# jianzhangcs/DAGL

Hardware: AMD Instinct MI355X
Metric: graph-attn fwd query-patches/s @256x256x64 k=8 (higher is better)
Workload: dtype f32

## Files before the change

### dagl_amd/csrc/aggregate.hip

```cpp
#include "dagl_common.h"
#include "aggregate_direct.h"
#include "topk_merge.h"

namespace dagl {


__global__ __launch_bounds__(256) void edge_softmax_fast_kernel(EdgeArgs a) {
    const int lane = threadIdx.x & 63;
    const size_t ql = (size_t)blockIdx.x * 4 + (threadIdx.x >> 6);
    if (ql >= (size_t)a.B * a.L) return;
    int n = a.cnt[ql];
    if (n > DAGL_FAST_CAP) n = DAGL_FAST_CAP;
    int key = 0x7fffffff; float s = 0.f;
    if (lane < n) { key = a.list_idx[ql * DAGL_FAST_CAP + lane]; s = a.list_val[ql * DAGL_FAST_CAP + lane]; }
#pragma unroll
    for (int k2 = 2; k2 <= 64; k2 <<= 1) {
#pragma unroll
        for (int j = k2 >> 1; j > 0; j >>= 1) {
            const int okey = __shfl_xor(key, j);
            const float os = __shfl_xor(s, j);
            const bool up = ((lane & k2) == 0);
            const bool lower = ((lane & j) == 0);
            const bool take = (lower == up) ? (okey < key) : (okey > key);
            if (take) { key = okey; s = os; }
// ... 52 lines not shown
__global__ void row_stats_kernel(size_t n_rows, const float* __restrict__ nb_wgt, const int32_t* __restrict__ nb_cnt,
                                 const int64_t* __restrict__ row_off, int width, int32_t* __restrict__ deg,
                                 float* __restrict__ rowsum) {
    const size_t r = (size_t)blockIdx.x * blockDim.x + threadIdx.x;
    if (r >= n_rows) return;
    const int n = nb_cnt[r];
    if (n < 0) return;
    const float* w = nb_wgt + (row_off ? (size_t)row_off[r] : r * width);
    double s = 0.0;
    for (int j = 0; j < n; ++j) s += (double)w[j];
    if (deg) deg[r] = n;
    if (rowsum) rowsum[r] = (float)s;
}

int launch_row_stats(hipStream_t s, size_t n_rows, const float* nb_wgt, const int32_t* nb_cnt, const int64_t* row_off,
                     int width, int32_t* deg, float* rowsum) {
    hipLaunchKernelGGL(row_stats_kernel, dim3((unsigned)((n_rows + 255) / 256)), dim3(256), 0, s, n_rows, nb_wgt,
                       nb_cnt, row_off, width, deg, rowsum);
    DAGL_LAUNCH_CHECK("row_stats_kernel");
    return DAGL_OK;
}

int launch_edge_softmax(hipStream_t s, const EdgeArgs& a) {
    const size_t nq = (size_t)a.B * a.L;
    dim3 grid((unsigned)((nq + 3) / 4)), block(256);
    if (a.mode == DAGL_MODE_ADAPTIVE) {
        if (a.row_off == nullptr) hipLaunchKernelGGL(edge_softmax_fast_kernel, grid, block, 0, s, a);
        else hipLaunchKernelGGL(edge_softmax_csr_kernel, grid, block, 0, s, a);
    } else {
        const int ks = topk_slots(a.k);
        if (a.splits * 2 * ks > TOPK_MAX_CAND) {
            set_error("edge softmax: %d candidates per query exceed %d", a.splits * 2 * ks, TOPK_MAX_CAND);
            return DAGL_ERR_INVALID;
        }
        dim3 g2 = grid;
        if (a.run_flags != nullptr && g2.x > 128) g2.x = 128;
        hipLaunchKernelGGL(edge_softmax_topk_kernel, g2, block, 0, s, a, ks, grid.x);
    }
    DAGL_LAUNCH_CHECK("edge_softmax_kernel");
    return DAGL_OK;
}

__global__ __launch_bounds__(256) void aggregate_direct_kernel(AggArgs a) {
    __shared__ int sh_of[AGG_STAGE];
    __shared__ float sh_w[AGG_STAGE];
    aggregate_direct_block(a, blockIdx.y, blockIdx.x, sh_of, sh_w);
}

int launch_aggregate_direct(hipStream_t s, const AggArgs& a) {
    dim3 grid((unsigned)a.g.L, a.B), block(256);
    hipLaunchKernelGGL(aggregate_direct_kernel, grid, block, 0, s, a);
    DAGL_LAUNCH_CHECK("aggregate_direct_kernel");
    return DAGL_OK;
}

template <int KU>
__global__ __launch_bounds__(256) void gather_rows_kernel(int L, int k, int P4, const int32_t* __restrict__ idx,
                                                          const float* __restrict__ wgt,
                                                          const float4* __restrict__ values,
                                                          float4* __restrict__ out) {
    const size_t t = (size_t)blockIdx.x * blockDim.x + threadIdx.x;
    if (t >= (size_t)L * P4) return;
    const int q = (int)(t / P4), r = (int)(t % P4);
    const int32_t* ip = idx + (size_t)q * k;
    const float* wp = wgt + (size_t)q * k;
    float4 acc = make_float4(0.f, 0.f, 0.f, 0.f);
    int j = 0;
    for (; j + KU <= k; j += KU) {
        int id[KU]; float w[KU]; float4 v[KU];
#pragma unroll
        for (int u = 0; u < KU; ++u) { id[u] = ip[j + u]; w[u] = wp[j + u]; }
#pragma unroll
        for (int u = 0; u < KU; ++u) {
            const bool ok = id[u] >= 0;
            v[u] = values[(size_t)(ok ? id[u] : 0) * P4 + r];
            if (!ok) w[u] = 0.f;
        }
#pragma unroll
        for (int u = 0; u < KU; ++u) {
            acc.x = fmaf(w[u], v[u].x, acc.x); acc.y = fmaf(w[u], v[u].y, acc.y);
            acc.z = fmaf(w[u], v[u].z, acc.z); acc.w = fmaf(w[u], v[u].w, acc.w);
        }
    }
    for (; j < k; ++j) {
        const int id = ip[j];
        if (id < 0) continue;
        const float w = wp[j];
        const float4 v = values[(size_t)id * P4 + r];
        acc.x = fmaf(w, v.x, acc.x); acc.y = fmaf(w, v.y, acc.y);
        acc.z = fmaf(w, v.z, acc.z); acc.w = fmaf(w, v.w, acc.w);
    }
    out[t] = acc;
}

int launch_gather_fixed(hipStream_t s, int L, int k, int P_, const int32_t* idx, const float* wgt,
                        const float* values, float* out) {
    const int P4 = P_ / 4;
    const size_t items = (size_t)L * P4;
    dim3 grid((unsigned)((items + 255) / 256)), block(256);
    if (k % 8 == 0)
        hipLaunchKernelGGL(gather_rows_kernel<8>, grid, block, 0, s, L, k, P4, idx, wgt,
                           reinterpret_cast<const float4*>(values), reinterpret_cast<float4*>(out));
    else
        hipLaunchKernelGGL(gather_rows_kernel<4>, grid, block, 0, s, L, k, P4, idx, wgt,
                           reinterpret_cast<const float4*>(values), reinterpret_cast<float4*>(out));
    DAGL_LAUNCH_CHECK("gather_rows_kernel");
    return DAGL_OK;
}

__global__ __launch_bounds__(256) void fold_kernel(Grid g, const float* __restrict__ agg, float* __restrict__ out,
                                                   int imgs, int heads, RangeTag range) {
    const int b = blockIdx.z;
    const int y = blockIdx.y;
    const int x = blockIdx.x * blockDim.x + threadIdx.x;
    const bool poisoned = (range.word != nullptr && *range.word == range.tag) || (range.veto != nullptr && *range.veto == range.tag);
    if (range.done != nullptr && b == 0 && y == 0 && blockIdx.x == 0 && threadIdx.x == 0) *range.done = range.tag;
    if (x >= g.W) return;
    int r0 = (y - 3 + QS - 1) / QS; if (y - 3 < 0) r0 = 0;
    int r1 = (y + 3) / QS; if (r1 > g.Lh - 1) r1 = g.Lh - 1;
    int c0 = (x - 3 + QS - 1) / QS; if (x - 3 < 0) c0 = 0;
    int c1 = (x + 3) / QS; if (c1 > g.Lw - 1) c1 = g.Lw - 1;
    float4 acc[CH / 4];
#pragma unroll
    for (int u = 0; u < CH / 4; ++u) acc[u] = make_float4(0.f, 0.f, 0.f, 0.f);
    for (int r = r0; r <= r1; ++r) {
        const int kh = y - (QS * r - 3);
        for (int c = c0; c <= c1; ++c) {
            const int kw = x - (QS * c - 3);
            const float4* p = reinterpret_cast<const float4*>(
                agg + ((size_t)b * g.L + (size_t)r * g.Lw + c) * P + (kh * KS + kw) * CH);
#pragma unroll
            for (int u = 0; u < CH / 4; ++u) {
                const float4 v = p[u];
                acc[u].x += v.x; acc[u].y += v.y; acc[u].z += v.z; acc[u].w += v.w;
            }
        }
    }
    float cnt = (float)((r1 - r0 + 1) * (c1 - c0 + 1));
    if (poisoned) cnt = __builtin_nanf("");
    const int head = b / imgs, img = b - head * imgs;
    float* o = out + ((size_t)img * heads + head) * CH * g.N + (size_t)y * g.W + x;
#pragma unroll
    for (int u = 0; u < CH / 4; ++u) {
        o[(size_t)(4 * u + 0) * g.N] = acc[u].x / cnt;
        o[(size_t)(4 * u + 1) * g.N] = acc[u].y / cnt;
        o[(size_t)(4 * u + 2) * g.N] = acc[u].z / cnt;
        o[(size_t)(4 * u + 3) * g.N] = acc[u].w / cnt;
    }
}

__device__ __forceinline__ void key_row_col(int id, int W, float inv_w, int& jy, int& jx) {
    jy = (int)((float)id * inv_w);
    jx = id - jy * W;
    if (jx < 0) { --jy; jx += W; } else if (jx >= W) { ++jy; jx -= W; }
}

__global__ __launch_bounds__(256) void aggregate_fold_kernel(AggArgs a, float* __restrict__ out, int imgs, int heads,
                                                             RangeTag range) {
    const Grid& g = a.g;
    const int b = blockIdx.z;
    const int t = blockIdx.x * blockDim.x + threadIdx.x;
    const int pix = t >> 2, u = t & 3;
    bool poisoned = range.word != nullptr && *range.word == range.tag;
    if (range.done != nullptr && b == 0 && blockIdx.x == 0 && threadIdx.x == 0) *range.done = range.tag;
    if (a.unserved != nullptr && *a.unserved != 0) {
        poisoned = true;
        if (b == 0 && blockIdx.x == 0 && threadIdx.x == 0) *a.unserved_sticky = 1;
    }
    if (pix >= g.N) return;
    const int y = pix / g.W, x = pix - y * g.W;
    int r0 = (y - 3 + QS - 1) / QS; if (y - 3 < 0) r0 = 0;
    int r1 = (y + 3) / QS; if (r1 > g.Lh - 1) r1 = g.Lh - 1;
    int c0 = (x - 3 + QS - 1) / QS; if (x - 3 < 0) c0 = 0;
    int c1 = (x + 3) / QS; if (c1 > g.Lw - 1) c1 = g.Lw - 1;
    const float4* vm = reinterpret_cast<const float4*>(a.b2p + (size_t)b * g.Hp * g.Wp * CH) + u;
    const int W = g.W, Wp = g.Wp;
    const float inv_w = 1.0f / (float)W;
    float4 acc = make_float4(0.f, 0.f, 0.f, 0.f);
    for (int r = r0; r <= r1; ++r) {
        const int kh = y - (QS * r - 3);
        for (int c = c0; c <= c1; ++c) {
            const int kw = x - (QS * c - 3);
            const size_t ql = (size_t)b * g.L + (size_t)r * g.Lw + c;
            const int n = a.nb_cnt[ql];
            const int32_t* ip = a.nb_idx + ql * a.width;
            const float* wp = a.nb_wgt + ql * a.width;
            float4 q = make_float4(0.f, 0.f, 0.f, 0.f);
            int j = 0;
            for (; j + 4 <= n; j += 4) {
                int id[4]; float w[4]; float4 v[4];
#pragma unroll
                for (int e = 0; e < 4; ++e) { id[e] = ip[j + e]; w[e] = wp[j + e]; }
#pragma unroll
                for (int e = 0; e < 4; ++e) {
                    int jy, jx; key_row_col(id[e], W, inv_w, jy, jx);
                    v[e] = vm[((jy + kh) * Wp + jx + kw) * (CH / 4)];
                }
#pragma unroll
                for (int e = 0; e < 4; ++e) {
                    q.x = fmaf(w[e], v[e].x, q.x); q.y = fmaf(w[e], v[e].y, q.y);
                    q.z = fmaf(w[e], v[e].z, q.z); q.w = fmaf(w[e], v[e].w, q.w);
                }
            }
            for (; j < n; ++j) {
                const int id = ip[j]; const float w = wp[j];
                int jy, jx; key_row_col(id, W, inv_w, jy, jx);
                const float4 v = vm[((jy + kh) * Wp + jx + kw) * (CH / 4)];
                q.x = fmaf(w, v.x, q.x); q.y = fmaf(w, v.y, q.y);
                q.z = fmaf(w, v.z, q.z); q.w = fmaf(w, v.w, q.w);
            }
            acc.x += q.x; acc.y += q.y; acc.z += q.z; acc.w += q.w;
        }
    }
    float cnt = (float)((r1 - r0 + 1) * (c1 - c0 + 1));
    if (poisoned) cnt = __builtin_nanf("");
    const int head = b / imgs, img = b - head * imgs;
    float* o = out + ((size_t)img * heads + head) * CH * g.N + (size_t)y * g.W + x;
    o[(size_t)(4 * u + 0) * g.N] = acc.x / cnt;
    o[(size_t)(4 * u + 1) * g.N] = acc.y / cnt;
    o[(size_t)(4 * u + 2) * g.N] = acc.z / cnt;
    o[(size_t)(4 * u + 3) * g.N] = acc.w / cnt;
}

int launch_aggregate_fold(hipStream_t s, const AggArgs& a, float* out, int heads, RangeTag range) {
    dim3 grid((unsigned)(((size_t)a.g.N * 4 + 255) / 256), 1, a.B), block(256);
    hipLaunchKernelGGL(aggregate_fold_kernel, grid, block, 0, s, a, out, a.B / heads, heads, range);
    DAGL_LAUNCH_CHECK("aggregate_fold_kernel");
    return DAGL_OK;
}

int launch_fold(hipStream_t s, int B, const Grid& g, const float* agg, float* out, int heads, RangeTag range) {
    dim3 grid((g.W + 63) / 64, g.H, B), block(64);
    hipLaunchKernelGGL(fold_kernel, grid, block, 0, s, g, agg, out, B / heads, heads, range);
    DAGL_LAUNCH_CHECK("fold_kernel");
    return DAGL_OK;
}

constexpr int MIX_TILES = 4;
__global__ __launch_bounds__(256) void stage_mix_kernel(int HW, const float* __restrict__ cat, const float* __restrict__ x,
                                                        const float* __restrict__ mix_w, const float* __restrict__ mix_b,
                                                        float* __restrict__ out) {
    const int lane = threadIdx.x & 63, wave = threadIdx.x >> 6;
    const int i = lane & 15, g = lane >> 4;
    const int b = blockIdx.y;
    const int pw = (blockIdx.x * 4 + wave) * (16 * MIX_TILES);
    if (pw >= HW) return;
    float w[4][16];
#pragma unroll
    for (int n = 0; n < 4; ++n)
#pragma unroll
        for (int T = 0; T < 16; ++T) w[n][T] = mix_w[(n * 16 + i) * 64 + 4 * T + g];
    float bo[4][4];
#pragma unroll
    for (int n = 0; n < 4; ++n)
#pragma unroll
        for (int r = 0; r < 4; ++r) bo[n][r] = mix_b[n * 16 + 4 * g + r];
    float av[MIX_TILES][16];
#pragma unroll
    for (int t = 0; t < MIX_TILES; ++t) {
        int px = pw + 16 * t + i; if (px >= HW) px = HW - 1;
        const float* cb = cat + (size_t)b * 64 * HW + px;
#pragma unroll
        for (int T = 0; T < 16; ++T) av[t][T] = cb[(size_t)(4 * T + g) * HW];
    }
#pragma unroll
    for (int t = 0; t < MIX_TILES; ++t) {
        f32x4 acc[4];
#pragma unroll
        for (int n = 0; n < 4; ++n) acc[n] = (f32x4){0.f, 0.f, 0.f, 0.f};
#pragma unroll
        for (int T = 0; T < 16; ++T)
#pragma unroll
            for (int n = 0; n < 4; ++n) acc[n] = __builtin_amdgcn_mfma_f32_16x16x4f32(w[n][T], av[t][T], acc[n], 0, 0, 0);
        const int pp = pw + 16 * t + i;
#pragma unroll
        for (int n = 0; n < 4; ++n) {
#pragma unroll
            for (int r = 0; r < 4; ++r) {
                const int o = n * 16 + 4 * g + r;
                if (pp < HW) {
                    const size_t idx = ((size_t)b * 64 + o) * HW + pp;
                    out[idx] = (acc[n][r] + bo[n][r]) + x[idx];
                }
            }
        }
    }
}

int launch_stage_mix(hipStream_t s, int B, int HW, const float* cat, const float* x, const float* mix_w,
                     const float* mix_b, float* out) {
    dim3 grid((HW + 64 * MIX_TILES - 1) / (64 * MIX_TILES), B), block(256);
    hipLaunchKernelGGL(stage_mix_kernel, grid, block, 0, s, HW, cat, x, mix_w, mix_b, out);
    DAGL_LAUNCH_CHECK("stage_mix_kernel");
    return DAGL_OK;
}

}
```

### dagl_amd/csrc/screen.hip

```cpp
#include "dagl_common.h"

namespace dagl {

typedef __bf16 bf16x8 __attribute__((ext_vector_type(8)));
typedef short s16x8 __attribute__((ext_vector_type(8)));

constexpr int SK = 64;
constexpr int STEP_ELEMS = SK * DSH;
constexpr int STEP_PIECES = 27;
constexpr int KB = 13;
constexpr float DELTA = SCREEN_DELTA;
constexpr int GKEEP = 4;

__device__ __forceinline__ float theta_of_sampled_max(float m) { return m > 0.f ? m * ((1.0f - SCREEN_DELTA) / (1.0f + SCREEN_DELTA)) : 0.f; }

__device__ __forceinline__ void screen_spill(const ScreenArgs& a, size_t qlin, int key, float sv) {
    const unsigned pos = atomicAdd(a.spill_cnt + qlin, 1u);
    if (pos < (unsigned)SCREEN_SPILL) a.spill[qlin * SCREEN_SPILL + pos] = make_int2(key, __float_as_int(sv));
}

__device__ __forceinline__ void load_query_fragments(const ScreenArgs& a, int b, int q0, int qc, int lane, bf16x8 (&qf)[KB]) {
    const int h = lane >> 5;
    int t0 = q0; if (t0 > ((a.L - 1) & ~31)) t0 = (a.L - 1) & ~31;
    const int i = lane & 31;
// ... 459 lines not shown
                }
            }
            if (qvalid[w]) *reinterpret_cast<float4*>(a.gmax + seg[w] * GKEEP) = make_float4(top[0], top[1], top[2], top[3]);
        } else {
            if ((VAR & 16) && gm[w][0] == 12345.f) n_loc[w] = 1;
            if (qvalid[w]) cseg[w][-(a.splits * 2)] = make_int2(n_loc[w], SMAX ? __float_as_int(smx[w]) : 0);
        }
    }
    if (!(VAR & 64)) dbg_stamp(a.times, blockIdx.y * gridDim.x + blockIdx.x, 3);
#ifdef DAGL_ABLATION
    if ((VAR & 128) && a.times != nullptr && tid == 0) a.times[(size_t)(blockIdx.y * gridDim.x + blockIdx.x) * 4 + 3] = clk1 - clk0;
#endif
}

__global__ void adaptive_theta_kernel(size_t n, const float* __restrict__ mt, const float* __restrict__ bs,
                                      float* __restrict__ theta, int both) {
    const size_t i = (size_t)blockIdx.x * blockDim.x + threadIdx.x;
    if (i >= n) return;
    const float ta = adaptive_theta_of(mt[i], bs[i]);
    theta[i] = both ? fmaxf(ta, theta[i]) : ta;
}

int launch_adaptive_theta(hipStream_t s, size_t n, const float* mt, const float* bs, float* theta, bool both) {
    hipLaunchKernelGGL(adaptive_theta_kernel, dim3((unsigned)((n + 255) / 256)), dim3(256), 0, s, n, mt, bs, theta, both ? 1 : 0);
    DAGL_LAUNCH_CHECK("adaptive_theta_kernel");
    return DAGL_OK;
}

int launch_screen(hipStream_t s, const ScreenArgs& a, int pass) {
    const int qblock = (a.qblock == 512 || a.qblock == 384) ? a.qblock : 256;
    const int n_qgroups = (a.L + qblock - 1) / qblock;
    dim3 grid(n_qgroups * a.splits, a.B);
    if (pass == 1 && a.seg_max) {
        if (qblock == 512) hipLaunchKernelGGL((screen_ring_kernel<1, 16, 0, 1, true>), grid, dim3(1024), 0, s, a, n_qgroups);
        else if (qblock == 384) hipLaunchKernelGGL((screen_ring_kernel<1, 12, 0, 1, true>), grid, dim3(768), 0, s, a, n_qgroups);
        else hipLaunchKernelGGL((screen_kernel<1, 1, 0, 256, true>), grid, dim3(512), 0, s, a, n_qgroups);
        DAGL_LAUNCH_CHECK("screen_kernel");
        return DAGL_OK;
    }
#define SCR_RING(P_, W_, V_) hipLaunchKernelGGL((screen_ring_kernel<P_, W_, V_>), grid, dim3(W_ * 64), 0, s, args, n_qgroups)
#define SCR_BARRIER(P_, V_) hipLaunchKernelGGL((screen_kernel<P_, 1, V_>), grid, dim3(512), 0, s, args, n_qgroups)
#ifdef DAGL_ABLATION
    const size_t n_blk = (size_t)grid.x * grid.y;
    const bool ring_phases = a.variant == 64 && qblock == 512;
    ScreenArgs args = a; args.times = (getenv("DAGL_TIMES_FILE") && pass == 1) ? dbg_times_buffer(ring_phases ? n_blk * 20 : n_blk) : nullptr;
#define SCR_RV(P_) switch (a.variant) { case 0: SCR_RING(P_, 16, 0); break; case 1: SCR_RING(P_, 16, 1); break; case 2: SCR_RING(P_, 16, 2); break; case 3: SCR_RING(P_, 16, 3); break; \
                                             case 7: SCR_RING(P_, 16, 7); break; case 15: SCR_RING(P_, 16, 15); break; case 31: SCR_RING(P_, 16, 31); break; case 6: SCR_RING(P_, 16, 6); break; \
                                             case 18: SCR_RING(P_, 16, 18); break; case 8: SCR_RING(P_, 16, 8); break; case 64: SCR_RING(P_, 16, 64); break; \
                                             case 4: SCR_RING(P_, 16, 4); break; case 16: SCR_RING(P_, 16, 16); break; case 5: SCR_RING(P_, 16, 5); break; case 20: SCR_RING(P_, 16, 20); break; \
                                             case 17: SCR_RING(P_, 16, 17); break; case 21: SCR_RING(P_, 16, 21); break; \
                                             case 128: SCR_RING(P_, 16, 128); break; case 159: SCR_RING(P_, 16, 159); break; case 144: SCR_RING(P_, 16, 144); break; case 130: SCR_RING(P_, 16, 130); break; \
                                             case 145: SCR_RING(P_, 16, 145); break; case 149: SCR_RING(P_, 16, 149); break; default: SCR_RING(P_, 16, 0); break; }
#define SCR_VARIANTS(P_)                                               \
    switch (a.variant) {                                                 \
        case 0: SCR_BARRIER(P_, 0); break;                               \
        case 1: SCR_BARRIER(P_, 1); break;                               \
        case 2: SCR_BARRIER(P_, 2); break;                               \
        case 4: SCR_BARRIER(P_, 4); break;                               \
        case 8: SCR_BARRIER(P_, 8); break;                               \
        case 16: SCR_BARRIER(P_, 16); break;                             \
        case 40: SCR_BARRIER(P_, 40); break;                             \
        case 9: SCR_BARRIER(P_, 9); break;                               \
        case 41: SCR_BARRIER(P_, 41); break;                             \
        case 32: SCR_BARRIER(P_, 32); break;                             \
        case 48: SCR_BARRIER(P_, 48); break;                             \
        case 24: SCR_BARRIER(P_, 24); break;                             \
        case 25: SCR_BARRIER(P_, 25); break;                             \
        case 57: SCR_BARRIER(P_, 57); break;                             \
        case 23: SCR_BARRIER(P_, 23); break;                             \
        case 39: SCR_BARRIER(P_, 39); break;                             \
        case 55: SCR_BARRIER(P_, 55); break;                             \
        case 15: SCR_BARRIER(P_, 15); break;                             \
        case 63: SCR_BARRIER(P_, 63); break;                             \
        case 121: SCR_BARRIER(P_, 121); break;                           \
        case 89: SCR_BARRIER(P_, 89); break;                             \
        case 73: SCR_BARRIER(P_, 73); break;                             \
        case 72: SCR_BARRIER(P_, 72); break;                             \
        default: SCR_BARRIER(P_, 7); break;                              \
    }
#else
    const ScreenArgs& args = a;
#define SCR_RV(P_) SCR_RING(P_, 16, 0);
#define SCR_VARIANTS(P_) SCR_BARRIER(P_, 0);
#endif
    if (qblock == 512) {
        if (pass == 0) SCR_RING(0, 16, 0); else { SCR_RV(1) }
    } else if (qblock == 384) {
        if (pass == 0) SCR_RING(0, 12, 0); else SCR_RING(1, 12, 0);
    } else {
        if (pass == 0) { SCR_VARIANTS(0) } else { SCR_VARIANTS(1) }
    }
#ifdef DAGL_ABLATION
    if (args.times) dbg_times_dump(s, ring_phases ? "screen_ring_kernel<1>_phases" : (qblock == 256 ? "screen_kernel<1>" : "screen_ring_kernel<1>"), args.times, ring_phases ? n_blk * 20 : n_blk);
#endif
    DAGL_LAUNCH_CHECK("screen_kernel");
    return DAGL_OK;
}

constexpr int THETA_PER_LANE = 8;
__global__ __launch_bounds__(256) void screen_theta_kernel(int n_rows, int G, int k, const float* __restrict__ gmax,
                                                           float* __restrict__ theta, const int32_t* gate, unsigned* __restrict__ spill_cnt) {
    if (gate != nullptr && *gate == 0) return;
    const int lane = threadIdx.x & 63;
    const size_t row = (size_t)blockIdx.x * 4 + (threadIdx.x >> 6);
    if (row >= (size_t)n_rows) return;
    if (spill_cnt != nullptr && lane == 0) spill_cnt[row] = 0u;
    float v[THETA_PER_LANE];
#pragma unroll
    for (int u = 0; u < THETA_PER_LANE; ++u) {
        const int t = lane + 64 * u;
        v[u] = (t < G) ? gmax[row * G + t] : -1.0f;
    }
    float kth = -1.0f;
    for (int r = 0; r < k; ++r) {
        float lm = v[0];
#pragma unroll
        for (int u = 1; u < THETA_PER_LANE; ++u) lm = fmaxf(lm, v[u]);
        const float wm = wave_max_f32(lm);
        kth = wm;
        if (wm < 0.f) break;
        const unsigned long long bal = __ballot(lm == wm);
        const int owner = __ffsll((long long)bal) - 1;
        bool taken = false;
#pragma unroll
        for (int u = 0; u < THETA_PER_LANE; ++u) {
            const bool hit = (lane == owner) && !taken && (v[u] == wm);
            v[u] = hit ? -1.0f : v[u];
            taken = taken || hit;
        }
    }
    if (lane == 0) theta[row] = (kth > 0.f) ? kth * ((1.0f - DELTA) / (1.0f + DELTA)) : 0.0f;
}

int launch_screen_theta(hipStream_t s, int n_rows, int G, int k, const float* gmax, float* theta, const int32_t* gate, unsigned* spill_cnt) {
    if (G > 64 * THETA_PER_LANE) { set_error("screen_theta: %d groups exceed %d", G, 64 * THETA_PER_LANE); return DAGL_ERR_INVALID; }
    hipLaunchKernelGGL(screen_theta_kernel, dim3((n_rows + 3) / 4), dim3(256), 0, s, n_rows, G, k, gmax, theta, gate, spill_cnt);
    DAGL_LAUNCH_CHECK("screen_theta_kernel");
    return DAGL_OK;
}

constexpr int RF_MAX_CAND = 1024;
constexpr int RF_ROUNDS_MAX_K = 16;

__device__ __forceinline__ float rf_logit(float s, float mtq, float bsq, bool adaptive) {
    float m = 1.0f;
    if (adaptive) m = (s - mtq) + bsq;
    return __fmul_rn(__fmul_rn(s, m), SOFTMAX_SCALE);
}

__device__ __forceinline__ bool rf_before(float va, int ka, float vb, int kb) {
    return (va > vb) || (va == vb && ka < kb);
}

constexpr int RF_HEAVY_WAVES = 8;
constexpr int RF_HEAVY_MIN = 64;
constexpr int RF_HEAVY_CAP = 1024;
template <bool HEAVY>
__device__ __forceinline__ void refine_query(const RefineArgs& a, const size_t ql, int* __restrict__ ci, float* __restrict__ cv,
                                             int* sh_total) {
    const int lane = threadIdx.x & 63, w = threadIdx.x >> 6;
    const bool lead = !HEAVY || w == 0;
    const int b = (int)(ql / a.L);
    const int S2 = a.splits * 2;
    bool overflow = false;
    const int grp = lane >> 3, gl = lane & 7;
    const float* qrow = a.wq + ((size_t)b * a.rows_q + (ql - (size_t)b * a.L)) * DS;
    float4 qv[7];
#pragma unroll
    for (int u = 0; u < 7; ++u) {
        const int c4 = gl + 8 * u;
        const float4 raw = *reinterpret_cast<const float4*>(qrow + 4 * (c4 < D / 4 ? c4 : D / 4 - 1));
        qv[u] = (c4 < D / 4) ? raw : make_float4(0.f, 0.f, 0.f, 0.f);
    }

    const bool adaptive = (a.mode != DAGL_MODE_TOPK);
    const float thq = (a.mode != DAGL_MODE_ADAPTIVE) ? a.theta[ql] : 0.f;
    const float mtq = adaptive ? a.mt[ql] : 0.f, bsq = adaptive ? a.bs[ql] : 0.f;

    int total = 0;
    if (lead)
    for (int s0 = 0; s0 < S2; s0 += 64) {
        const int sgi = s0 + lane;
        const bool sv = sgi < S2;
        const int2* rec = a.cand + ql * (size_t)a.capseg * S2 + (sv ? sgi : 0);
        const int2 r0 = rec[0], c0 = rec[S2], c1 = rec[2 * (size_t)S2], c2 = rec[3 * (size_t)S2];
        int cnt = sv ? r0.x : 0;
        if (cnt > a.capseg - 1) { overflow = true; cnt = a.capseg - 1; }
        const int incl = wave_scan_incl_i32(cnt);
        const int off = total + incl - cnt;
        if (off + cnt > RF_MAX_CAND) { overflow = true; cnt = max(0, RF_MAX_CAND - off); }
        if (cnt > 0) { ci[off] = c0.x; cv[off] = __int_as_float(c0.y); }
        if (cnt > 1) { ci[off + 1] = c1.x; cv[off + 1] = __int_as_float(c1.y); }
        if (cnt > 2) { ci[off + 2] = c2.x; cv[off + 2] = __int_as_float(c2.y); }
        for (int e = 3; e < cnt; ++e) {
            const int2 c = rec[(size_t)(1 + e) * S2];
            ci[off + e] = c.x; cv[off + e] = __int_as_float(c.y);
        }
        total += __builtin_amdgcn_readlane(incl, 63);
    }
    overflow = __any(overflow);
    if (lead && a.spill != nullptr && overflow) {
        const unsigned sc_n = a.spill_cnt[ql];
        if (sc_n > 0u) {
            if (sc_n <= (unsigned)SCREEN_SPILL && total + (int)sc_n <= RF_MAX_CAND) {
                const bool seg_only = !(total >= RF_MAX_CAND);
                for (unsigned e = lane; e < sc_n; e += 64) {
                    const int2 c = a.spill[ql * SCREEN_SPILL + e];
                    ci[total + e] = c.x; cv[total + e] = __int_as_float(c.y);
                }
                total += (int)sc_n;
                if (seg_only) overflow = false;
            } else overflow = true;
        }
    }
    if (total > RF_MAX_CAND) total = RF_MAX_CAND;
    if (a.mode == DAGL_MODE_ADAPTIVE && a.ovf_list != nullptr && total > 2 * a.width) { overflow = true; total = 0; }
    __threadfence_block();
    if (HEAVY) {
        if (w == 0 && lane == 0) *sh_total = total;
        __syncthreads();
        total = *sh_total;
    } else if (a.mode == DAGL_MODE_ADAPTIVE && a.heavy_list != nullptr && total >= RF_HEAVY_MIN) {
        int pos = RF_HEAVY_CAP;
        if (lane == 0) { pos = atomicAdd(a.heavy_count, 1); if (pos < RF_HEAVY_CAP) a.heavy_list[pos] = (int32_t)ql; }
        if (__shfl(pos, 0) < RF_HEAVY_CAP) return;
    }

    constexpr int TU = 4;
    if (a.mode != DAGL_MODE_ADAPTIVE && total > a.k && total <= 64 * TU) {
        int key[TU]; float ub[TU], work[TU];
#pragma unroll
        for (int u = 0; u < TU; ++u) {
            const int c = lane + 64 * u;
            const bool have = c < total;
            key[u] = have ? ci[c] : -1;
            const float sv = have ? cv[c] : 0.f;
            ub[u] = fabsf(sv);
            work[u] = have ? ((sv >= 0.f) ? sv : thq) : -1.0f;
        }
        float tk = -1.0f;
        if (!HEAVY && a.k > RF_ROUNDS_MAX_K) {
            unsigned uw[TU];
#pragma unroll
            for (int u = 0; u < TU; ++u) uw[u] = work[u] > 0.f ? __float_as_uint(work[u]) : 0u;
            unsigned prefix = 0u;
            for (int bit = 30; bit >= 0; --bit) {
                const unsigned t = prefix | (1u << bit);
                int cnt = 0;
#pragma unroll
                for (int u = 0; u < TU; ++u) cnt += uw[u] >= t ? 1 : 0;
                if (wave_sum_i32(cnt) >= a.k) prefix = t;
            }
            tk = __uint_as_float(prefix);
        } else
        for (int r = 0; r < a.k; ++r) {
            float lm = work[0];
#pragma unroll
            for (int u = 1; u < TU; ++u) lm = fmaxf(lm, work[u]);
            const float wm = wave_max_f32(lm);
            tk = wm;
            const unsigned long long bal = __ballot(lm == wm);
            const int owner = __ffsll((long long)bal) - 1;
            bool taken = false;
#pragma unroll
            for (int u = 0; u < TU; ++u) {
                const bool hit = (lane == owner) && !taken && (work[u] == wm);
                work[u] = hit ? -2.0f : work[u];
                taken = taken || hit;
            }
        }
        const float cut = tk * ((1.0f - DELTA) / (1.0f + DELTA)) * (1.0f - 1e-6f);
        int base = 0;
#pragma unroll
        for (int u = 0; u < TU; ++u) {
            const bool keep = key[u] >= 0 && ub[u] >= cut;
            const unsigned long long bal = __ballot(keep);
            const int pos = base + __popcll(bal & ((1ull << lane) - 1ull));
            if (keep) ci[pos] = key[u];
            base += __popcll(bal);
        }
        total = base;
        __threadfence_block();
    } else if (a.mode != DAGL_MODE_ADAPTIVE && total > a.k) {
        const int nu = (total + 63) >> 6;
        unsigned taken = 0u;
        float tk = -1.0f;
        if (!HEAVY && a.k > RF_ROUNDS_MAX_K) {
            unsigned uw[RF_MAX_CAND / 64];
#pragma unroll
            for (int u = 0; u < RF_MAX_CAND / 64; ++u) {
                const int c = lane + 64 * u;
                float lbv = 0.f;
                if (u < nu && c < total) { const float sv = cv[c]; lbv = (sv >= 0.f) ? sv : thq; }
                uw[u] = lbv > 0.f ? __float_as_uint(lbv) : 0u;
            }
            unsigned prefix = 0u;
            for (int bit = 30; bit >= 0; --bit) {
                const unsigned t = prefix | (1u << bit);
                int cnt = 0;
#pragma unroll
                for (int u = 0; u < RF_MAX_CAND / 64; ++u) cnt += uw[u] >= t ? 1 : 0;
                if (wave_sum_i32(cnt) >= a.k) prefix = t;
            }
            tk = __uint_as_float(prefix);
        } else
        for (int r = 0; r < a.k; ++r) {
            float lm = -1.0f; int lu = -1;
            for (int u = 0; u < nu; ++u) {
                const int c = lane + 64 * u;
                if (c < total && !((taken >> u) & 1u)) {
                    const float sv = cv[c];
                    const float lbv = (sv >= 0.f) ? sv : thq;
                    if (lbv > lm) { lm = lbv; lu = u; }
                }
            }
            const float wm = wave_max_f32(lm);
            tk = wm;
            const unsigned long long bal = __ballot(lu >= 0 && lm == wm);
            if (bal != 0ull && lane == __ffsll((long long)bal) - 1) taken |= 1u << lu;
        }
        const float cut = tk * ((1.0f - DELTA) / (1.0f + DELTA)) * (1.0f - 1e-6f);
        int base = 0;
        for (int u = 0; u < nu; ++u) {
            const int c = lane + 64 * u;
            const bool have = c < total;
            const int key = have ? ci[c] : -1;
            const float ub = have ? fabsf(cv[c]) : 0.f;
            const bool keep = key >= 0 && ub >= cut;
            const unsigned long long bal = __ballot(keep);
            const int pos = base + __popcll(bal & ((1ull << lane) - 1ull));
            if (keep) ci[pos] = key;
            base += __popcll(bal);
        }
        total = base;
        __threadfence_block();
    }

    if (!HEAVY) dbg_stamp(a.times, blockIdx.x, 1);
    const float* xb = a.x + (size_t)b * a.rows_x * DS;
#pragma unroll 2
    for (int c0 = HEAVY ? 8 * w : 0; c0 < total; c0 += HEAVY ? 8 * RF_HEAVY_WAVES : 8) {
        const int c = c0 + grp;
        const bool okc = c < total;
        int key = okc ? ci[c] : 0;
        const bool inb = key < a.N;
        if (!inb) key = 0;
        const float* xrow = xb + (size_t)key * DS;
        float4 xv[7];
#pragma unroll
        for (int u = 0; u < 7; ++u) {
            const int c4 = gl + 8 * u;
            xv[u] = *reinterpret_cast<const float4*>(xrow + 4 * (c4 < D / 4 ? c4 : 0));
// ... 55 lines not shown
            v = cv[lane]; key = ci[lane];
            if (key < 0 || (a.mode == DAGL_MODE_ADAPTIVE_TOPK && !(((v - mtq) + bsq) > 0.f))) { v = -3.0f; key = 0x7fffffff; }
        }
        int rank = 0;
        for (int j = 0; j < total; ++j) {
            const float vj = __int_as_float(__builtin_amdgcn_readlane(__float_as_int(v), j)); const int kj = __builtin_amdgcn_readlane(key, j);
            rank += rf_before(vj, kj, v, key) ? 1 : 0;
        }
        const unsigned long long valid_mask = __ballot(v > -2.0f);
        n = min(a.k, (int)__popcll(valid_mask));
        if (v > -2.0f && rank < n) { my_s[0] = v; my_key[0] = key; pos0 = rank; }
        else pos0 = -1;
    } else {
        if (a.mode == DAGL_MODE_ADAPTIVE_TOPK) {
            for (int c = lane; c < total; c += 64)
                if (!(((cv[c] - mtq) + bsq) > 0.f)) ci[c] = -1;
            __threadfence_block();
        }
        for (int r = 0; r < a.k; ++r) {
            float bv = -2.f; int bi = 0x7fffffff, bpos = -1;
            for (int t = lane; t < total; t += 64) {
                const float v = cv[t]; const int id = ci[t];
                if (id >= 0 && (v > bv || (v == bv && id < bi))) { bv = v; bi = id; bpos = t; }
            }
#pragma unroll
            for (int o = 32; o > 0; o >>= 1) {
                const float ov = __shfl_xor(bv, o); const int oi = __shfl_xor(bi, o); const int op = __shfl_xor(bpos, o);
                if (ov > bv || (ov == bv && oi < bi)) { bv = ov; bi = oi; bpos = op; }
            }
            if (bpos < 0) break;
            if (lane == r) { my_s[0] = bv; my_key[0] = bi; }
            if (lane == 0) ci[bpos] = -1;
            __threadfence_block();
            ++n;
        }
    }

    float lg[RU];
    double M = -1e300;
#pragma unroll
    for (int u = 0; u < RU; ++u) {
        const int e = (u == 0) ? pos0 : lane + 64 * u;
        const bool valid = e >= 0 && e < n;
        lg[u] = valid ? rf_logit(my_s[u], mtq, bsq, adaptive) : 0.f;
        if (valid) M = fmax(M, (double)lg[u]);
    }
    M = wave_max_f64(M);
    if (n < a.N) M = fmax(M, 0.0);
    double ev[RU], sum = 0.0;
#pragma unroll
    for (int u = 0; u < RU; ++u) {
        const int e = (u == 0) ? pos0 : lane + 64 * u;
        ev[u] = (e >= 0 && e < n) ? exp((double)lg[u] - M) : 0.0;
        sum += ev[u];
    }
    sum = wave_sum_f64(sum);
    sum += (double)(a.N - n) * exp(-M);
#pragma unroll
    for (int u = 0; u < RU; ++u) {
        const int e = (u == 0) ? pos0 : lane + 64 * u;
        if (e >= 0 && e < n) {
            a.nb_idx[ql * a.width + e] = my_key[u];
            a.nb_wgt[ql * a.width + e] = (float)(ev[u] / sum);
            if (a.nb_s != nullptr) a.nb_s[ql * a.width + e] = my_s[u];
        }
    }
    int ovf_pos = -1;
    if (lane == 0) {
        a.nb_cnt[ql] = (overflow && a.ovf_list != nullptr) ? -1 : n;
        if (overflow) {
            const size_t qg = (size_t)b * a.n_qgroups_exact + (size_t)(ql - (size_t)b * a.L) / 128;
            a.redo_flags[qg] = 1;
            atomicAdd(reinterpret_cast<unsigned long long*>(&a.stats[STAT_FLAGGED]), 1ull);
            if (a.ovf_list != nullptr) {
                ovf_pos = atomicAdd(a.ovf_count, 1);
                if (ovf_pos < a.ovf_cap) a.ovf_list[ovf_pos] = (int32_t)ql;
            }
        }
    }
    if (overflow && a.ovf_list != nullptr && a.ovf_qrows != nullptr) {
        ovf_pos = __shfl(ovf_pos, 0);
        if (ovf_pos < a.ovf_cap)
            for (int c = lane; c < DS; c += 64) a.ovf_qrows[(size_t)ovf_pos * DS + c] = qrow[c];
    }
}

__global__ __launch_bounds__(256) void refine_kernel(RefineArgs a) {
    __shared__ int c_idx[4][RF_MAX_CAND];
    __shared__ float c_val[4][RF_MAX_CAND];
    if (a.gate != nullptr && *a.gate == 0) return;
    if (a.policy != nullptr && *a.policy != 0) a.capseg = a.capseg_tight;
    const int w = threadIdx.x >> 6;
    dbg_stamp(a.times, blockIdx.x, 0);
    const size_t ql = (size_t)blockIdx.x * 4 + w;
    if (ql >= (size_t)a.B * a.L) return;
    refine_query<false>(a, ql, c_idx[w], c_val[w], nullptr);
    dbg_stamp(a.times, blockIdx.x, 3);
}

__global__ __launch_bounds__(64 * RF_HEAVY_WAVES) void refine_heavy_kernel(RefineArgs a) {
    __shared__ int c_idx[RF_MAX_CAND];
    __shared__ float c_val[RF_MAX_CAND];
    __shared__ int sh_total;
    const int n = min(*a.heavy_count, RF_HEAVY_CAP);
    for (int slot = blockIdx.x; slot < n; slot += gridDim.x) {
        refine_query<true>(a, (size_t)a.heavy_list[slot], c_idx, c_val, &sh_total);
        __syncthreads();
    }
}

constexpr float DN_BOUND_OK = 12.0f;
__device__ __forceinline__ float rm_logit(float sc, float mtq, float bsq) {
    const float m = (sc - mtq) + bsq;
    return m > 0.f ? __fmul_rn(__fmul_rn(sc, m), SOFTMAX_SCALE) : 0.f;
}
__global__ __launch_bounds__(256) void rowmax_exact_kernel(RefineArgs a, float* __restrict__ smax) {
    __shared__ int c_idx[4][RF_MAX_CAND];
    __shared__ float c_val[4][RF_MAX_CAND];
    const int lane = threadIdx.x & 63, w = threadIdx.x >> 6;
    const size_t ql = (size_t)blockIdx.x * 4 + w;
    if (ql >= (size_t)a.B * a.L) return;
    int* ci = c_idx[w]; float* cv = c_val[w];
    const int b = (int)(ql / a.L);
    const int S2 = a.splits * 2;
    const float thq = theta_of_sampled_max(a.theta[ql]);
    float sm = 0.f;
    bool overflow = false;
    int total = 0;
    for (int s0 = 0; s0 < S2; s0 += 64) {
        const int sgi = s0 + lane;
        const int2 hdr = (sgi < S2) ? a.cand[ql * (size_t)a.capseg * S2 + sgi] : make_int2(0, 0);
        if (hdr.x > 0) sm = fmaxf(sm, __int_as_float(hdr.y));
        if (hdr.x > a.capseg - 1) overflow = true;
        total += wave_sum_i32(min(hdr.x, a.capseg - 1));
    }
    sm = wave_max_f32(sm);
    overflow = __any(overflow) || total > RF_MAX_CAND;
    const float s_hi = sm * (1.0f / (1.0f - DELTA)) * (1.0f + 1e-6f), s_lo = sm * (1.0f / (1.0f + DELTA));
    const float mtq = a.mt[ql], bsq = a.bs[ql];
    if (overflow || rm_logit(s_hi, mtq, bsq) - rm_logit(s_lo, mtq, bsq) <= DN_BOUND_OK) {
        if (lane == 0) smax[ql] = s_hi;
        return;
    }
    const int grp = lane >> 3, gl = lane & 7;
    const float* qrow = a.wq + ((size_t)b * a.rows_q + (ql - (size_t)b * a.L)) * DS;
    float4 qv[7];
#pragma unroll
    for (int u = 0; u < 7; ++u) {
        const int c4 = gl + 8 * u;
        const float4 raw = *reinterpret_cast<const float4*>(qrow + 4 * (c4 < D / 4 ? c4 : D / 4 - 1));
        qv[u] = (c4 < D / 4) ? raw : make_float4(0.f, 0.f, 0.f, 0.f);
    }
    total = 0;
    for (int s0 = 0; s0 < S2; s0 += 64) {
        const int sgi = s0 + lane;
        const bool sv = sgi < S2;
        const int2* rec = a.cand + ql * (size_t)a.capseg * S2 + (sv ? sgi : 0);
        const int cnt = sv ? rec[0].x : 0;
        const int incl = wave_scan_incl_i32(cnt);
        const int off = total + incl - cnt;
        for (int e = 0; e < cnt; ++e) {
            const int2 c = rec[(size_t)(1 + e) * S2];
            ci[off + e] = c.x; cv[off + e] = __int_as_float(c.y);
        }
        total += __builtin_amdgcn_readlane(incl, 63);
    }
    __threadfence_block();
    float lb = -1.0f;
    for (int c = lane; c < total; c += 64) { const float sv = cv[c]; lb = fmaxf(lb, (sv >= 0.f) ? sv : thq); }
    lb = wave_max_f32(lb);
    const float cut = lb * ((1.0f - DELTA) / (1.0f + DELTA)) * (1.0f - 1e-6f);
    int base = 0;
    for (int c0 = 0; c0 < total; c0 += 64) {
        const int c = c0 + lane;
        const bool have = c < total;
        const int key = have ? ci[c] : -1;
        const bool keep = have && fabsf(cv[c]) >= cut && key < a.N;
        const unsigned long long bal = __ballot(keep);
        const int pos = base + __popcll(bal & ((1ull << lane) - 1ull));
        if (keep) ci[pos] = key;
        base += __popcll(bal);
    }
    total = base;
    __threadfence_block();
    const float* xb = a.x + (size_t)b * a.rows_x * DS;
    double best = 0.0;
#pragma unroll 2
    for (int c0 = 0; c0 < total; c0 += 8) {
        const int c = c0 + grp;
        const bool okc = c < total;
        const float* xrow = xb + (size_t)(okc ? ci[c] : 0) * DS;
        float4 xv[7];
#pragma unroll
        for (int u = 0; u < 7; ++u) {
            const int c4 = gl + 8 * u;
            xv[u] = *reinterpret_cast<const float4*>(xrow + 4 * (c4 < D / 4 ? c4 : 0));
        }
        double acc = 0.0;
#pragma unroll
        for (int u = 0; u < 7; ++u)
            acc += (double)qv[u].x * (double)xv[u].x + (double)qv[u].y * (double)xv[u].y +
                   (double)qv[u].z * (double)xv[u].z + (double)qv[u].w * (double)xv[u].w;
        acc += dpp_zero_d<0xB1>(acc); acc += dpp_zero_d<0x4E>(acc); acc += dpp_zero_d<0x141>(acc);
        if (okc && gl == 0) best = fmax(best, acc);
    }
    best = wave_max_f64(best);
    if (lane == 0) smax[ql] = (float)best;
}

int launch_rowmax_exact(hipStream_t s, const RefineArgs& a, float* smax) {
    if (a.splits * 2 > RF_MAX_CAND) { set_error("rowmax_exact: too many segments"); return DAGL_ERR_INVALID; }
    const size_t nq = (size_t)a.B * a.L;
    hipLaunchKernelGGL(rowmax_exact_kernel, dim3((unsigned)((nq + 3) / 4)), dim3(256), 0, s, a, smax);
    DAGL_LAUNCH_CHECK("rowmax_exact_kernel");
    return DAGL_OK;
}

__global__ __launch_bounds__(1024) void degree_stats_kernel(size_t n_rows, const int32_t* __restrict__ nb_cnt,
                                                            int64_t* __restrict__ stats, int count_over) {
    __shared__ long long ssum[16];
    __shared__ int smax[16], sover[16];
    long long sum = 0; int mx = 0, over = 0;
    for (size_t r = threadIdx.x; r < n_rows; r += blockDim.x) {
        const int d = nb_cnt[r]; sum += d; mx = max(mx, d); over += (count_over > 0 && d > count_over) ? 1 : 0;
    }
#pragma unroll
    for (int o = 32; o > 0; o >>= 1) { sum += __shfl_xor(sum, o); mx = max(mx, __shfl_xor(mx, o)); over += __shfl_xor(over, o); }
    if ((threadIdx.x & 63) == 0) { ssum[threadIdx.x >> 6] = sum; smax[threadIdx.x >> 6] = mx; sover[threadIdx.x >> 6] = over; }
    __syncthreads();
    if (threadIdx.x == 0) {
        long long t = 0; int m = 0, ov = 0;
        for (int w = 0; w < (int)(blockDim.x >> 6); ++w) { t += ssum[w]; m = max(m, smax[w]); ov += sover[w]; }
        stats[STAT_EDGES] = t; stats[STAT_MAX_DEGREE] = m;
        if (count_over > 0) stats[STAT_FLAGGED] = ov;
    }
}

int launch_degree_stats(hipStream_t s, size_t n_rows, const int32_t* nb_cnt, int64_t* stats, int count_over) {
    hipLaunchKernelGGL(degree_stats_kernel, dim3(1), dim3(1024), 0, s, n_rows, nb_cnt, stats, count_over);
    DAGL_LAUNCH_CHECK("degree_stats_kernel");
    return DAGL_OK;
}

int launch_refine(hipStream_t s, const RefineArgs& a) {
    if (a.splits * 2 * a.capseg > RF_MAX_CAND && a.splits * 2 > RF_MAX_CAND) {
        set_error("refine: too many segments"); return DAGL_ERR_INVALID;
    }
    const size_t nq = (size_t)a.B * a.L;
#ifdef DAGL_ABLATION
    RefineArgs at = a; at.times = getenv("DAGL_TIMES_FILE") ? dbg_times_buffer((nq + 3) / 4) : nullptr;
    hipLaunchKernelGGL(refine_kernel, dim3((unsigned)((nq + 3) / 4)), dim3(256), 0, s, at);
    if (at.times) dbg_times_dump(s, "refine_kernel", at.times, (nq + 3) / 4);
#else
    hipLaunchKernelGGL(refine_kernel, dim3((unsigned)((nq + 3) / 4)), dim3(256), 0, s, a);
#endif
    DAGL_LAUNCH_CHECK("refine_kernel");
    if (a.heavy_list != nullptr && a.mode == DAGL_MODE_ADAPTIVE) {
        hipLaunchKernelGGL(refine_heavy_kernel, dim3(256), dim3(64 * RF_HEAVY_WAVES), 0, s, a);
        DAGL_LAUNCH_CHECK("refine_heavy_kernel");
    }
    return DAGL_OK;
}
int refine_heavy_cap() { return RF_HEAVY_CAP; }

__global__ __launch_bounds__(256) void topk_policy_kernel(int64_t* stats, int32_t* policy, int32_t* gate, int32_t* redo_flags, int n_flags,
                                                          long long n_queries) {
    __shared__ int go, n_groups;
    if (threadIdx.x == 0) n_groups = 0;
    __syncthreads();
    if (*policy == 0 && stats[STAT_FLAGGED] > 0) {
        int loc = 0;
        for (int e = threadIdx.x; e < n_flags; e += blockDim.x) loc += redo_flags[e] != 0 ? 1 : 0;
        if (loc) atomicAdd(&n_groups, loc);
    }
    __syncthreads();
    if (threadIdx.x == 0) go = (*policy == 0 && (long long)n_groups * 50 > (long long)n_flags) ? 1 : 0;
    (void)n_queries;
    __syncthreads();
    if (!go) return;
    for (int e = threadIdx.x; e < n_flags; e += blockDim.x) redo_flags[e] = 0;
    __syncthreads();
    if (threadIdx.x == 0) { stats[STAT_EDGES] = 0; stats[STAT_MAX_DEGREE] = 0; stats[STAT_FLAGGED] = 0; *policy = 1; *gate = 1; }
}

int launch_topk_policy(hipStream_t s, int64_t* stats, int32_t* policy, int32_t* gate, int32_t* redo_flags, int n_flags, long long n_queries) {
    hipLaunchKernelGGL(topk_policy_kernel, dim3(1), dim3(256), 0, s, stats, policy, gate, redo_flags, n_flags, n_queries);
    DAGL_LAUNCH_CHECK("topk_policy_kernel");
    return DAGL_OK;
}

}
```

Measured before the change: 17.16 million.

## Redistribute fold aggregation across quad lanes and balance candidate gather across wave

The aggregate-fold kernel now has each of the four lanes in a quad load the neighbour list of one overlapping window, vectorised when aligned. DPP quad broadcasts then share offsets and weights so all lanes gather their own channel slice from every window in 8-wide batches. This replaces the serial per-window loops and is meant to raise memory-level parallelism and cut redundant index and weight loads. In the screen kernels, segment-record gathering preloads a configurable number of records per lane and spreads the leftover records evenly across the wave with a scan and binary search, instead of leaving long per-lane serial tails. The cost is extra shuffles and speculative loads, plus a second template instantiation of the fold kernel.

```diff
diff --git a/dagl_amd/csrc/aggregate.hip b/dagl_amd/csrc/aggregate.hip
--- a/dagl_amd/csrc/aggregate.hip
+++ b/dagl_amd/csrc/aggregate.hip
@@ -228,9 +228,61 @@
 __device__ __forceinline__ void key_row_col(int id, int W, float inv_w, int& jy, int& jx) {
     jy = (int)((float)id * inv_w);
     jx = id - jy * W;
-    if (jx < 0) { --jy; jx += W; } else if (jx >= W) { ++jy; jx -= W; }
-}
-
+    const int adj = (jx < 0) ? -1 : ((jx >= W) ? 1 : 0);
+    jy += adj; jx -= adj * W;
+}
+
+template <bool VEC>
+__device__ __forceinline__ void fold_list8(const int32_t* __restrict__ ip, const float* __restrict__ wp, const int j0,
+                                           const int width, unsigned (&id)[8], float (&w)[8]) {
+    if (VEC) {
+        const int j1 = (j0 + 4 < width) ? j0 + 4 : j0;
+        const int4 i0 = *reinterpret_cast<const int4*>(ip + j0), i1 = *reinterpret_cast<const int4*>(ip + j1);
+        const float4 w0 = *reinterpret_cast<const float4*>(wp + j0), w1 = *reinterpret_cast<const float4*>(wp + j1);
+        id[0] = i0.x; id[1] = i0.y; id[2] = i0.z; id[3] = i0.w; id[4] = i1.x; id[5] = i1.y; id[6] = i1.z; id[7] = i1.w;
+        w[0] = w0.x; w[1] = w0.y; w[2] = w0.z; w[3] = w0.w; w[4] = w1.x; w[5] = w1.y; w[6] = w1.z; w[7] = w1.w;
+    } else {
+#pragma unroll
+        for (int e = 0; e < 8; ++e) {
+            const int j = (j0 + e < width) ? j0 + e : width - 1;
+            id[e] = ip[j]; w[e] = wp[j];
+        }
+    }
+}
+
+template <int S>
+__device__ __forceinline__ int quad_bcast_i(int v) { return __builtin_amdgcn_update_dpp(0, v, S * 0x55, 0xf, 0xf, false); }
+template <int S>
+__device__ __forceinline__ float quad_bcast_f(float v) { return __int_as_float(quad_bcast_i<S>(__float_as_int(v))); }
+
+template <int S0>
+__device__ __forceinline__ void fold_window_pair(const char* __restrict__ vmb, const unsigned cg, const unsigned (&of)[8],
+                                                 const float (&w)[8], const int j0, const int na, const int nb, float4& qa,
+                                                 float4& qb) {
+    float4 va[8], vb[8];
+#pragma unroll
+    for (int e = 0; e < 8; ++e) va[e] = *reinterpret_cast<const float4*>(vmb + ((unsigned)quad_bcast_i<S0>((int)of[e]) + cg));
+#pragma unroll
+    for (int e = 0; e < 8; ++e) vb[e] = *reinterpret_cast<const float4*>(vmb + ((unsigned)quad_bcast_i<S0 + 1>((int)of[e]) + cg));
+#pragma unroll
+    for (int e = 0; e < 8; ++e) {
+        const float we = quad_bcast_f<S0>(w[e]);
+        if (j0 + e < na) {
+            qa.x = fmaf(we, va[e].x, qa.x); qa.y = fmaf(we, va[e].y, qa.y);
+            qa.z = fmaf(we, va[e].z, qa.z); qa.w = fmaf(we, va[e].w, qa.w);
+        }
+    }
+#pragma unroll
+    for (int e = 0; e < 8; ++e) {
+        const float we = quad_bcast_f<S0 + 1>(w[e]);
+        if (j0 + e < nb) {
+            qb.x = fmaf(we, vb[e].x, qb.x); qb.y = fmaf(we, vb[e].y, qb.y);
+            qb.z = fmaf(we, vb[e].z, qb.z); qb.w = fmaf(we, vb[e].w, qb.w);
+        }
+    }
+}
+
+template <bool VEC>
 __global__ __launch_bounds__(256) void aggregate_fold_kernel(AggArgs a, float* __restrict__ out, int imgs, int heads,
                                                              RangeTag range) {
     const Grid& g = a.g;
@@ -249,45 +301,44 @@
     int r1 = (y + 3) / QS; if (r1 > g.Lh - 1) r1 = g.Lh - 1;
     int c0 = (x - 3 + QS - 1) / QS; if (x - 3 < 0) c0 = 0;
     int c1 = (x + 3) / QS; if (c1 > g.Lw - 1) c1 = g.Lw - 1;
-    const float4* vm = reinterpret_cast<const float4*>(a.b2p + (size_t)b * g.Hp * g.Wp * CH) + u;
-    const int W = g.W, Wp = g.Wp;
+    const char* vmb = reinterpret_cast<const char*>(a.b2p + (size_t)b * g.Hp * g.Wp * CH);
+    const unsigned cg = (unsigned)(u * sizeof(float4));
+    const int W = g.W, Wp = g.Wp, width = a.width;
     const float inv_w = 1.0f / (float)W;
+    const int rr = r0 + (u >> 1), cc = c0 + (u & 1);
+    const bool have = rr <= r1 && cc <= c1;
+    const int r = have ? rr : r0, c = have ? cc : c0;
+    const size_t ql = (size_t)b * g.L + (size_t)r * g.Lw + c;
+    const int32_t* ip = a.nb_idx + ql * width;
+    const float* wp = a.nb_wgt + ql * width;
+    int n_own = a.nb_cnt[ql];
+    unsigned of[8]; float w[8];
+    fold_list8<VEC>(ip, wp, 0, width, of, w);
+    if (!have) n_own = 0;
+    const int wo = (y - (QS * r - 3)) * Wp + x - (QS * c - 3);
+    const int n0 = quad_bcast_i<0>(n_own), n1 = quad_bcast_i<1>(n_own), n2 = quad_bcast_i<2>(n_own), n3 = quad_bcast_i<3>(n_own);
+    const int nmax = max(max(n0, n1), max(n2, n3));
+    float4 q[4];
+#pragma unroll
+    for (int s = 0; s < 4; ++s) q[s] = make_float4(0.f, 0.f, 0.f, 0.f);
+#pragma unroll 1
+    for (int j0 = 0;;) {
+#pragma unroll
+        for (int e = 0; e < 8; ++e) {
+            int jy, jx; key_row_col(j0 + e < n_own ? (int)of[e] : 0, W, inv_w, jy, jx);
+            of[e] = (unsigned)(jy * Wp + jx + wo) * (unsigned)(CH * sizeof(float));
+        }
+        fold_window_pair<0>(vmb, cg, of, w, j0, n0, n1, q[0], q[1]);
+        asm volatile("" : "+v"(q[0].x), "+v"(q[0].y), "+v"(q[0].z), "+v"(q[0].w), "+v"(q[1].x), "+v"(q[1].y), "+v"(q[1].z), "+v"(q[1].w)
+                     :: "memory");
+        fold_window_pair<2>(vmb, cg, of, w, j0, n2, n3, q[2], q[3]);
+        j0 += 8;
+        if (j0 >= width || j0 >= nmax) break;
+        fold_list8<VEC>(ip, wp, j0, width, of, w);
+    }
     float4 acc = make_float4(0.f, 0.f, 0.f, 0.f);
-    for (int r = r0; r <= r1; ++r) {
-        const int kh = y - (QS * r - 3);
-        for (int c = c0; c <= c1; ++c) {
-            const int kw = x - (QS * c - 3);
-            const size_t ql = (size_t)b * g.L + (size_t)r * g.Lw + c;
-            const int n = a.nb_cnt[ql];
-            const int32_t* ip = a.nb_idx + ql * a.width;
-            const float* wp = a.nb_wgt + ql * a.width;
-            float4 q = make_float4(0.f, 0.f, 0.f, 0.f);
-            int j = 0;
-            for (; j + 4 <= n; j += 4) {
-                int id[4]; float w[4]; float4 v[4];
-#pragma unroll
-                for (int e = 0; e < 4; ++e) { id[e] = ip[j + e]; w[e] = wp[j + e]; }
-#pragma unroll
-                for (int e = 0; e < 4; ++e) {
-                    int jy, jx; key_row_col(id[e], W, inv_w, jy, jx);
-                    v[e] = vm[((jy + kh) * Wp + jx + kw) * (CH / 4)];
-                }
-#pragma unroll
-                for (int e = 0; e < 4; ++e) {
-                    q.x = fmaf(w[e], v[e].x, q.x); q.y = fmaf(w[e], v[e].y, q.y);
-                    q.z = fmaf(w[e], v[e].z, q.z); q.w = fmaf(w[e], v[e].w, q.w);
-                }
-            }
-            for (; j < n; ++j) {
-                const int id = ip[j]; const float w = wp[j];
-                int jy, jx; key_row_col(id, W, inv_w, jy, jx);
-                const float4 v = vm[((jy + kh) * Wp + jx + kw) * (CH / 4)];
-                q.x = fmaf(w, v.x, q.x); q.y = fmaf(w, v.y, q.y);
-                q.z = fmaf(w, v.z, q.z); q.w = fmaf(w, v.w, q.w);
-            }
-            acc.x += q.x; acc.y += q.y; acc.z += q.z; acc.w += q.w;
-        }
-    }
+#pragma unroll
+    for (int s = 0; s < 4; ++s) { acc.x += q[s].x; acc.y += q[s].y; acc.z += q[s].z; acc.w += q[s].w; }
     float cnt = (float)((r1 - r0 + 1) * (c1 - c0 + 1));
     if (poisoned) cnt = __builtin_nanf("");
     const int head = b / imgs, img = b - head * imgs;
@@ -300,7 +351,9 @@
 
 int launch_aggregate_fold(hipStream_t s, const AggArgs& a, float* out, int heads, RangeTag range) {
     dim3 grid((unsigned)(((size_t)a.g.N * 4 + 255) / 256), 1, a.B), block(256);
-    hipLaunchKernelGGL(aggregate_fold_kernel, grid, block, 0, s, a, out, a.B / heads, heads, range);
+    const bool vec = a.width % 4 == 0 && (((uintptr_t)a.nb_idx | (uintptr_t)a.nb_wgt) & 15) == 0;
+    if (vec) hipLaunchKernelGGL(aggregate_fold_kernel<true>, grid, block, 0, s, a, out, a.B / heads, heads, range);
+    else hipLaunchKernelGGL(aggregate_fold_kernel<false>, grid, block, 0, s, a, out, a.B / heads, heads, range);
     DAGL_LAUNCH_CHECK("aggregate_fold_kernel");
     return DAGL_OK;
 }
diff --git a/dagl_amd/csrc/screen.hip b/dagl_amd/csrc/screen.hip
--- a/dagl_amd/csrc/screen.hip
+++ b/dagl_amd/csrc/screen.hip
@@ -635,6 +635,65 @@
     return (va > vb) || (va == vb && ka < kb);
 }
 
+#ifndef DAGL_RF_FIRST
+#define DAGL_RF_FIRST 7
+#endif
+constexpr int RF_FIRST = DAGL_RF_FIRST;
+constexpr int RF_REST_BATCH = 4;
+template <int F>
+__device__ __forceinline__ int gather_segment_records(const int2* __restrict__ qrec, const int S2, const int capseg, const int s0,
+                                                      const int total, int* __restrict__ ci, float* __restrict__ cv,
+                                                      bool& overflow) {
+    const int lane = threadIdx.x & 63;
+    const int sgi = s0 + lane;
+    const bool sv = sgi < S2;
+    const int last = capseg - 1;
+    const int2* rec = qrec + (sv ? sgi : 0);
+    const int2 r0 = rec[0];
+    int2 c[F];
+#pragma unroll
+    for (int f = 0; f < F; ++f) c[f] = rec[(size_t)min(1 + f, last) * S2];
+    int cnt = sv ? r0.x : 0;
+    if (cnt > last) { overflow = true; cnt = last; }
+    const int incl = wave_scan_incl_i32(cnt);
+    const int off = total + incl - cnt;
+    if (off + cnt > RF_MAX_CAND) { overflow = true; cnt = max(0, RF_MAX_CAND - off); }
+#pragma unroll
+    for (int f = 0; f < F; ++f)
+        if (cnt > f) { ci[off + f] = c[f].x; cv[off + f] = __int_as_float(c[f].y); }
+    const int rem = max(cnt - F, 0);
+    if (__any(rem > 0)) {
+        const int rincl = wave_scan_incl_i32(rem);
+        const int rtot = __builtin_amdgcn_readlane(rincl, 63);
+        const int rexcl = rincl - rem;
+        const int dst0 = off + F - rexcl;
+        for (int j0 = 0; j0 < rtot; j0 += 64 * RF_REST_BATCH) {
+            int2 r[RF_REST_BATCH]; int dst[RF_REST_BATCH];
+#pragma unroll
+            for (int u = 0; u < RF_REST_BATCH; ++u) {
+                dst[u] = -1;
+                if (j0 + 64 * u < rtot) {
+                    const int j = j0 + 64 * u + lane;
+                    int sl = 0;
+#pragma unroll
+                    for (int step = 32; step > 0; step >>= 1)
+                        if (__shfl(rincl, sl + step - 1) <= j) sl += step;
+                    const bool ok = j < rtot;
+                    sl = ok ? sl : 0;
+                    const int e = j - __shfl(rexcl, sl);
+                    const int d = __shfl(dst0, sl) + j;
+                    r[u] = ok ? qrec[(size_t)(1 + F + e) * S2 + s0 + sl] : qrec[0];
+                    dst[u] = ok ? d : -1;
+                }
+            }
+#pragma unroll
+            for (int u = 0; u < RF_REST_BATCH; ++u)
+                if (dst[u] >= 0) { ci[dst[u]] = r[u].x; cv[dst[u]] = __int_as_float(r[u].y); }
+        }
+    }
+    return total + __builtin_amdgcn_readlane(incl, 63);
+}
+
 constexpr int RF_HEAVY_WAVES = 8;
 constexpr int RF_HEAVY_MIN = 64;
 constexpr int RF_HEAVY_CAP = 1024;
@@ -662,25 +721,8 @@
 
     int total = 0;
     if (lead)
-    for (int s0 = 0; s0 < S2; s0 += 64) {
-        const int sgi = s0 + lane;
-        const bool sv = sgi < S2;
-        const int2* rec = a.cand + ql * (size_t)a.capseg * S2 + (sv ? sgi : 0);
-        const int2 r0 = rec[0], c0 = rec[S2], c1 = rec[2 * (size_t)S2], c2 = rec[3 * (size_t)S2];
-        int cnt = sv ? r0.x : 0;
-        if (cnt > a.capseg - 1) { overflow = true; cnt = a.capseg - 1; }
-        const int incl = wave_scan_incl_i32(cnt);
-        const int off = total + incl - cnt;
-        if (off + cnt > RF_MAX_CAND) { overflow = true; cnt = max(0, RF_MAX_CAND - off); }
-        if (cnt > 0) { ci[off] = c0.x; cv[off] = __int_as_float(c0.y); }
-        if (cnt > 1) { ci[off + 1] = c1.x; cv[off + 1] = __int_as_float(c1.y); }
-        if (cnt > 2) { ci[off + 2] = c2.x; cv[off + 2] = __int_as_float(c2.y); }
-        for (int e = 3; e < cnt; ++e) {
-            const int2 c = rec[(size_t)(1 + e) * S2];
-            ci[off + e] = c.x; cv[off + e] = __int_as_float(c.y);
-        }
-        total += __builtin_amdgcn_readlane(incl, 63);
-    }
+    for (int s0 = 0; s0 < S2; s0 += 64)
+        total = gather_segment_records<RF_FIRST>(a.cand + ql * (size_t)a.capseg * S2, S2, a.capseg, s0, total, ci, cv, overflow);
     overflow = __any(overflow);
     if (lead && a.spill != nullptr && overflow) {
         const unsigned sc_n = a.spill_cnt[ql];
@@ -1042,19 +1084,8 @@
         qv[u] = (c4 < D / 4) ? raw : make_float4(0.f, 0.f, 0.f, 0.f);
     }
     total = 0;
-    for (int s0 = 0; s0 < S2; s0 += 64) {
-        const int sgi = s0 + lane;
-        const bool sv = sgi < S2;
-        const int2* rec = a.cand + ql * (size_t)a.capseg * S2 + (sv ? sgi : 0);
-        const int cnt = sv ? rec[0].x : 0;
-        const int incl = wave_scan_incl_i32(cnt);
-        const int off = total + incl - cnt;
-        for (int e = 0; e < cnt; ++e) {
-            const int2 c = rec[(size_t)(1 + e) * S2];
-            ci[off + e] = c.x; cv[off + e] = __int_as_float(c.y);
-        }
-        total += __builtin_amdgcn_readlane(incl, 63);
-    }
+    for (int s0 = 0; s0 < S2; s0 += 64)
+        total = gather_segment_records<RF_FIRST>(a.cand + ql * (size_t)a.capseg * S2, S2, a.capseg, s0, total, ci, cv, overflow);
     __threadfence_block();
     float lb = -1.0f;
     for (int c = lane; c < total; c += 64) { const float sv = cv[c]; lb = fmaxf(lb, (sv >= 0.f) ? sv : thq); }
```

Measured after the change: 17.17 million (median of 3 runs). Within noise of the previous version (+0.1%).
